# kserve/kserve

Measured on AMD Instinct MI355X. Metric: output tok/s, llama-3-8b /v1/completions decode, higher is better.
Workload: dtype bfloat16; 1 GPU; model=llama-3-8b, global_batch=1536, seq_len=512, parallelism=dp1, kv_block_size=16, hipgraph=True, kv_cache_dtype=auto

## Files before the change

### build_hip.py

```python
#!/usr/bin/env python3

import os
import subprocess
import sys

REPO = os.path.dirname(os.path.abspath(__file__))
CSRC = os.path.join(REPO, "kserve_amd", "ops", "csrc")
BUILD = os.path.join(REPO, "build", "hip")
OUT_SO = os.path.join(REPO, "kserve_amd_C.so")

HIPCC = os.environ.get("HIPCC", "/opt/rocm/bin/hipcc")
ARCH = os.environ.get("PYTORCH_ROCM_ARCH", "gfx950")

KERNEL_SOURCES = [
    "rmsnorm.hip",
    "layernorm.hip",
    "activation.hip",
    "rope.hip",
    "kv_cache.hip",
    "attention_decode.hip",
    "attention_prefill.hip",
    "sampling.hip",
    "skinny_gemm.hip",
    "w8_gemm.hip",
    "gemm8.hip",
    "mfma_probe.hip",
]


def run(cmd):
    print("+", " ".join(cmd), flush=True)
    subprocess.check_call(cmd)


def newer(src, dst):
    return not os.path.exists(dst) or os.path.getmtime(src) > os.path.getmtime(dst)


def build(force: bool = False) -> str:
    import torch
    import sysconfig

    os.makedirs(BUILD, exist_ok=True)
    torch_dir = os.path.dirname(torch.__file__)
    torch_inc = [
        os.path.join(torch_dir, "include"),
        os.path.join(torch_dir, "include", "torch", "csrc", "api", "include"),
    ]
    py_inc = sysconfig.get_paths()["include"]

    common_h = os.path.join(CSRC, "common.h")
    layouts_h = os.path.join(CSRC, "mfma_layouts.h")
    objs = []
    for src in KERNEL_SOURCES:
        src_path = os.path.join(CSRC, src)
        obj = os.path.join(BUILD, src.replace(".hip", ".o"))
        objs.append(obj)
        if force or newer(src_path, obj) or newer(common_h, obj) or newer(layouts_h, obj):
            run([
                HIPCC, "-c", src_path, "-o", obj,
                f"--offload-arch={ARCH}", "-O3", "-std=c++17", "-fPIC",
                "-ffast-math",
            ])

    bind_src = os.path.join(CSRC, "bindings.cpp")
    bind_obj = os.path.join(BUILD, "bindings.o")
    if force or newer(bind_src, bind_obj):
        cmd = [
            HIPCC, "-c", bind_src, "-o", bind_obj,
            "-O2", "-std=c++17", "-fPIC",
            "-D_GLIBCXX_USE_CXX11_ABI=1",
            "-DTORCH_EXTENSION_NAME=kserve_amd_C",
            "-DUSE_ROCM", "-D__HIP_PLATFORM_AMD__",
            "-DTORCH_API_INCLUDE_EXTENSION_H",
            f"-I{py_inc}",
        ]
        cmd += [f"-I{d}" for d in torch_inc]
        run(cmd)
    objs.append(bind_obj)

    if force or any(newer(o, OUT_SO) for o in objs):
        run([
            HIPCC, "-shared", "-o", OUT_SO, *objs,
            f"-L{os.path.join(torch_dir, 'lib')}",
            "-ltorch", "-ltorch_cpu", "-ltorch_python", "-lc10",
            "-ltorch_hip", "-lc10_hip", "-lamdhip64",
            f"-Wl,-rpath,{os.path.join(torch_dir, 'lib')}",
        ])
    print(f"built {OUT_SO}")
    return OUT_SO


if __name__ == "__main__":
    build(force="--force" in sys.argv)
```

### kserve_amd/ops/__init__.py

```python

from __future__ import annotations

from typing import Optional, Tuple

import torch

from kserve_amd.errors import NoNativeExtension
from kserve_amd.ops import torch_ref

_C = None
_IMPORT_ERROR: Optional[str] = None
try:
    import kserve_amd_C as _C
except ImportError as e:
    _IMPORT_ERROR = str(e)


def has_native() -> bool:
    return _C is not None


def _native(op: str):
    if _C is None:
        raise NoNativeExtension(op, f"(import error: {_IMPORT_ERROR})")
    return _C


def rms_norm(x: torch.Tensor, weight: torch.Tensor, eps: float) -> torch.Tensor:
    if x.is_cuda:
        out = torch.empty_like(x)
        _native("rms_norm").rms_norm(out, x, weight, eps)
        return out
    return torch_ref.rms_norm(x, weight, eps)


def fused_add_rms_norm(
    x: torch.Tensor, residual: torch.Tensor, weight: torch.Tensor, eps: float
) -> Tuple[torch.Tensor, torch.Tensor]:
    if x.is_cuda:
        _native("fused_add_rms_norm").fused_add_rms_norm(x, residual, weight, eps)
        return x, residual
    return torch_ref.fused_add_rms_norm(x, residual, weight, eps)


def silu_and_mul(x: torch.Tensor) -> torch.Tensor:
    if x.is_cuda:
        d = x.shape[-1] // 2
        out = torch.empty(
            (*x.shape[:-1], d), dtype=x.dtype, device=x.device
        )
        _native("silu_and_mul").silu_and_mul(out, x)
        return out
    return torch_ref.silu_and_mul(x)


def rotary_embedding(
    positions: torch.Tensor,
    q: torch.Tensor,
    k: torch.Tensor,
    cos_sin_cache: torch.Tensor,
) -> Tuple[torch.Tensor, torch.Tensor]:
    if q.is_cuda:
        _native("rotary_embedding").rotary_embedding(positions, q, k, cos_sin_cache)
        return q, k
    return torch_ref.rotary_embedding(positions, q, k, cos_sin_cache)


def reshape_and_cache(
    k: torch.Tensor,
    v: torch.Tensor,
    k_cache: torch.Tensor,
    v_cache: torch.Tensor,
    slot_mapping: torch.Tensor,
) -> None:
    if k.is_cuda:
        _native("reshape_and_cache").reshape_and_cache(
            k, v, k_cache, v_cache, slot_mapping
        )
        return
    torch_ref.reshape_and_cache(k, v, k_cache, v_cache, slot_mapping)


def paged_attention_decode(
    q: torch.Tensor,
    k_cache: torch.Tensor,
    v_cache: torch.Tensor,
    block_tables: torch.Tensor,
    context_lens: torch.Tensor,
    scale: float,
    out: Optional[torch.Tensor] = None,
    window: int = 0,
) -> torch.Tensor:
    if q.is_cuda:
        if out is None:
            out = torch.empty_like(q)
        _native("paged_attention_decode").paged_attention_decode(
            out, q, k_cache, v_cache, block_tables, context_lens, scale,
            window,
        )
        return out
    return torch_ref.paged_attention_decode(
        q, k_cache, v_cache, block_tables, context_lens, scale,
        window=window,
    )


def flash_prefill_varlen(
    q: torch.Tensor,
    k: torch.Tensor,
    v: torch.Tensor,
    cu_seqlens: torch.Tensor,
    max_seqlen: int,
    scale: float,
    window: int = 0,
) -> torch.Tensor:
    if q.is_cuda:
        out = torch.empty_like(q)
        _native("flash_prefill").flash_prefill_varlen(
            out, q, k, v, cu_seqlens, int(max_seqlen), scale,
            causal=True, window=window,
        )
        return out
    return torch_ref.flash_prefill_varlen(
        q, k, v, cu_seqlens, scale, causal=True, window=window
    )


def context_attention_varlen(
    q: torch.Tensor,
    k_cache: torch.Tensor,
    v_cache: torch.Tensor,
    block_tables: torch.Tensor,
    cu_seqlens_q: torch.Tensor,
    context_lens: torch.Tensor,
    max_q_len: int,
    scale: float,
    window: int = 0,
) -> torch.Tensor:
    if q.is_cuda:
        out = torch.empty_like(q)
        _native("context_prefill").context_prefill_varlen(
            out, q, k_cache, v_cache, block_tables, context_lens,
            cu_seqlens_q, int(max_q_len), scale, window
        )
        return out
    return torch_ref.context_attention_varlen(
        q, k_cache, v_cache, block_tables, cu_seqlens_q, context_lens, scale,
        window=window,
    )


def greedy_sample(logits: torch.Tensor) -> torch.Tensor:
    if logits.is_cuda:
        out = torch.empty(
            logits.shape[0], dtype=torch.int64, device=logits.device
        )
        _native("greedy_sample").greedy_sample(out, logits)
        return out
    return torch_ref.greedy_sample(logits)


def random_sample(
    logits: torch.Tensor,
    temperatures: torch.Tensor,
    top_p: torch.Tensor,
    top_k: torch.Tensor,
    seeds: Optional[torch.Tensor] = None,
    generator: Optional[torch.Generator] = None,
    min_p: Optional[torch.Tensor] = None,
) -> torch.Tensor:
    has_min_p = min_p is not None and bool((min_p > 0).any())
    if logits.is_cuda and seeds is not None and not has_min_p:
        out = torch.empty(
            logits.shape[0], dtype=torch.int64, device=logits.device
        )
        needs_trunc = bool((top_p < 1.0).any()) or bool((top_k > 0).any())
        if needs_trunc:
            _native("random_sample").topk_topp_sample(
                out, logits, temperatures, top_p, top_k.to(torch.int32), seeds
            )
        else:
            _native("random_sample").gumbel_sample(
                out, logits, temperatures, top_k.to(torch.int32), seeds
            )
        return out
    return torch_ref.random_sample(
        logits, temperatures, top_p, top_k, generator=generator, min_p=min_p
    )


def linear(x: torch.Tensor, weight: torch.Tensor, bias: Optional[torch.Tensor] = None) -> torch.Tensor:
    import torch.nn.functional as F

    if (
        _C is not None
        and x.is_cuda
        and bias is None
        and x.dim() == 2
        and 0 < x.shape[0] <= 64
        and weight.shape[0] % 64 == 0
        and weight.shape[0] <= 8192
        and weight.shape[1] % 64 == 0
        and weight.shape[1] <= 8192
        and x.stride(1) == 1
    ):
        out = torch.empty(
            (x.shape[0], weight.shape[0]), dtype=x.dtype, device=x.device
        )
        _C.skinny_gemm(out, x, weight)
        return out
    return F.linear(x, weight, bias)


W8_MAX_TOKENS = 128

_W8_SCRATCH: dict = {}


def w8_scratch_numel(out_features: int, in_features: int) -> int:
    return -(-out_features // 2) * in_features


def reserve_w8_scratch(device, out_features: int, in_features: int) -> None:
    device = torch.device(device)
    if device.type != "cuda":
        return
    if device.index is None:
        device = torch.device("cuda", torch.cuda.current_device())
    numel = w8_scratch_numel(out_features, in_features)
    buf = _W8_SCRATCH.get(device)
    if buf is None or buf.numel() < numel:
        _W8_SCRATCH[device] = None
        _W8_SCRATCH[device] = torch.empty(
            numel, dtype=torch.bfloat16, device=device
        )


def _w8_scratch(device, out_features: int, in_features: int) -> torch.Tensor:
    buf = _W8_SCRATCH.get(device)
    if buf is None or buf.numel() < w8_scratch_numel(out_features, in_features):
        if torch.cuda.is_current_stream_capturing():
            raise RuntimeError(
                "fp8 dequant scratch too small during graph capture; "
                "call ops.reserve_w8_scratch when the weight is quantized"
            )
        reserve_w8_scratch(device, out_features, in_features)
        buf = _W8_SCRATCH[device]
    return buf


def linear_w8(
    x: torch.Tensor,
    qweight: torch.Tensor,
    scale: torch.Tensor,
    bias: Optional[torch.Tensor] = None,
) -> torch.Tensor:
    if not x.is_cuda:
# ... 86 lines not shown
```

### kserve_amd/ops/csrc/attention_decode.hip

```cpp
#include "common.h"
#include "mfma_layouts.h"

#define NEG_INF (-1e30f)

namespace {

constexpr int PAGE = 16;
constexpr int NWAVES = 4;

typedef __bf16 bf16x2v_t __attribute__((ext_vector_type(2)));

template <int D, int HPW, int OCC = 1, bool PB = false, bool D2 = false,
          bool V4 = false, bool MQ = false>
__global__ __launch_bounds__(256, OCC) void paged_attention_kernel(
    short* __restrict__ out,
    const short* __restrict__ q,
    const short* __restrict__ k_cache,
    const short* __restrict__ v_cache,
    const int* __restrict__ block_tables,
    const int* __restrict__ context_lens,
    const float scale,
    const int num_kv_heads,
    const int group,
    const int max_blocks,
// ... 798 lines not shown
        }
      }
    }
  }

#pragma unroll
  for (int g = 0; g < GROUP; ++g) {
    if (lane == 0) {
      lds_ml[wave][g][0] = m[g];
      lds_ml[wave][g][1] = l[g];
    }
#pragma unroll
    for (int a = 0; a < ACC; ++a)
      lds_acc[wave][g][lane * ACC + a] = acc[g][a];
  }
  __syncthreads();
  for (int g = wave; g < GROUP; g += NWAVES) {
    float m_all = NEG_INF;
#pragma unroll
    for (int w = 0; w < NWAVES; ++w) m_all = fmaxf(m_all, lds_ml[w][g][0]);
    float l_all = 0.f;
    float a_all[ACC];
#pragma unroll
    for (int a = 0; a < ACC; ++a) a_all[a] = 0.f;
#pragma unroll
    for (int w = 0; w < NWAVES; ++w) {
      const float wgt = __expf(lds_ml[w][g][0] - m_all);
      l_all += wgt * lds_ml[w][g][1];
#pragma unroll
      for (int a = 0; a < ACC; ++a)
        a_all[a] += wgt * lds_acc[w][g][lane * ACC + a];
    }
    const int head = kv_head * GROUP + g;
    if (n_splits == 1) {
      const float inv_l = (l_all > 0.f) ? 1.f / l_all : 0.f;
      short* op = out + ((long)seq * num_heads + head) * D + lane * ACC;
#pragma unroll
      for (int a = 0; a < ACC; ++a)
        op[a] = float_to_bf16_bits(a_all[a] * inv_l);
    } else {
      float* po = part_out +
                  (((long)seq * num_heads + head) * n_splits + split) * D +
                  lane * ACC;
#pragma unroll
      for (int a = 0; a < ACC; ++a) po[a] = a_all[a];
      if (lane == 0) {
        float* ml =
            part_ml + (((long)seq * num_heads + head) * n_splits + split) * 2;
        ml[0] = m_all;
        ml[1] = l_all;
      }
    }
  }
}

template <int D>
__global__ void paged_attention_reduce_kernel(
    short* __restrict__ out,
    const float* __restrict__ part_out,
    const float* __restrict__ part_ml,
    const long total_sh, const int n_splits) {
  constexpr int ACC = D / 64;
  const long sh = blockIdx.x * (long)(blockDim.x >> 6) + (threadIdx.x >> 6);
  const int lane = threadIdx.x & 63;
  if (sh >= total_sh) return;
  const float* ml_base = part_ml + sh * n_splits * 2;
  float m = NEG_INF;
  for (int sp = 0; sp < n_splits; ++sp) m = fmaxf(m, ml_base[sp * 2]);
  float l = 0.f;
  float acc[ACC];
#pragma unroll
  for (int a = 0; a < ACC; ++a) acc[a] = 0.f;
  for (int sp = 0; sp < n_splits; ++sp) {
    const float ms = ml_base[sp * 2];
    const float ls = ml_base[sp * 2 + 1];
    if (ls <= 0.f || ms <= NEG_INF) continue;
    const float w = __expf(ms - m);
    l += ls * w;
    const float* po = part_out + (sh * n_splits + sp) * D + lane * ACC;
#pragma unroll
    for (int a = 0; a < ACC; ++a) acc[a] += w * po[a];
  }
  const float inv_l = (l > 0.f) ? 1.f / l : 0.f;
  short* op = out + sh * D + lane * ACC;
#pragma unroll
  for (int a = 0; a < ACC; ++a) op[a] = float_to_bf16_bits(acc[a] * inv_l);
}

}


namespace {
inline hipError_t launch_split_reduce(void* out, void* part_out,
                                      void* part_ml, int num_seqs,
                                      int num_heads, int head_dim,
                                      int n_splits, hipStream_t stream) {
  if (n_splits <= 1) return hipSuccess;
  const long sh = (long)num_seqs * num_heads;
  const int wpb = 4;
  dim3 rgrid((unsigned)((sh + wpb - 1) / wpb));
  if (head_dim == 128) {
    hipLaunchKernelGGL((paged_attention_reduce_kernel<128>), rgrid,
                       dim3(wpb * 64), 0, stream, (short*)out,
                       (const float*)part_out, (const float*)part_ml, sh,
                       n_splits);
  } else {
    hipLaunchKernelGGL((paged_attention_reduce_kernel<64>), rgrid,
                       dim3(wpb * 64), 0, stream, (short*)out,
                       (const float*)part_out, (const float*)part_ml, sh,
                       n_splits);
  }
  HIP_CHECK_KERNEL();
  return hipSuccess;
}
}

extern "C" hipError_t ks_paged_attention_decode_fp8(
    void* out, const void* q, const void* k_cache, const void* v_cache,
    const void* block_tables, const void* context_lens, float scale,
    int num_seqs, int num_heads, int num_kv_heads, int head_dim,
    int max_blocks, int block_size, long q_row_stride, int n_splits,
    void* part_out, void* part_ml, int window, hipStream_t stream) {
  if (block_size != PAGE || head_dim != 128) return hipErrorInvalidValue;
  const int group = num_heads / num_kv_heads;
  if (group > NWAVES) return hipErrorInvalidValue;
  if (n_splits < 1) n_splits = 1;
  dim3 grid(num_kv_heads, num_seqs, n_splits);
  static const bool cvtb = [] {
    const char* e = getenv("KS_FP8_CVTB");
    return e == nullptr || e[0] != '0';
  }();
  if (cvtb) {
    hipLaunchKernelGGL((paged_attention_fp8_kernel<128, true>), grid,
                       dim3(256), 0, stream, (short*)out, (const short*)q,
                       (const unsigned char*)k_cache,
                       (const unsigned char*)v_cache,
                       (const int*)block_tables, (const int*)context_lens,
                       scale, num_kv_heads, group, max_blocks, q_row_stride,
                       n_splits, (float*)part_out, (float*)part_ml, window);
  } else {
    hipLaunchKernelGGL((paged_attention_fp8_kernel<128, false>), grid,
                       dim3(256), 0, stream, (short*)out, (const short*)q,
                       (const unsigned char*)k_cache,
                       (const unsigned char*)v_cache,
                       (const int*)block_tables, (const int*)context_lens,
                       scale, num_kv_heads, group, max_blocks, q_row_stride,
                       n_splits, (float*)part_out, (float*)part_ml, window);
  }
  HIP_CHECK_KERNEL();
  return launch_split_reduce(out, part_out, part_ml, num_seqs, num_heads,
                             head_dim, n_splits, stream);
}

extern "C" hipError_t ks_paged_attention_decode(
    void* out, const void* q, const void* k_cache, const void* v_cache,
    const void* block_tables, const void* context_lens, float scale,
    int num_seqs, int num_heads, int num_kv_heads, int head_dim,
    int max_blocks, int block_size, long q_row_stride, int n_splits,
    void* part_out, void* part_ml, int window, hipStream_t stream) {
  if (block_size != PAGE) return hipErrorInvalidValue;
  const int group = num_heads / num_kv_heads;
  const int hpw = (group + NWAVES - 1) / NWAVES;
  if (hpw > 2) return hipErrorInvalidValue;
  if (n_splits < 1) n_splits = 1;
  dim3 grid(num_kv_heads, num_seqs, n_splits);
  dim3 block(256);

  static const bool use_ws = [] {
    const char* e = getenv("KS_ATTN_WS");
    return e != nullptr && e[0] == '1';
  }();
  const bool pow2_group =
      group == 1 || group == 2 || group == 4 || group == 8;
  if (use_ws && pow2_group && head_dim == 128) {
#define LAUNCH_WS(GG)                                                       \
  hipLaunchKernelGGL((paged_attention_ws_kernel<128, GG>), grid, block, 0,  \
                     stream, (short*)out, (const short*)q,                  \
                     (const short*)k_cache, (const short*)v_cache,          \
                     (const int*)block_tables, (const int*)context_lens,    \
                     scale, num_kv_heads, max_blocks, q_row_stride,         \
                     n_splits, (float*)part_out, (float*)part_ml, window)
    if (group == 1) LAUNCH_WS(1);
    else if (group == 2) LAUNCH_WS(2);
    else if (group == 4) LAUNCH_WS(4);
    else LAUNCH_WS(8);
#undef LAUNCH_WS
    HIP_CHECK_KERNEL();
    return launch_split_reduce(out, part_out, part_ml, num_seqs, num_heads,
                               head_dim, n_splits, stream);
  }

  static const bool use_h2 = [] {
    const char* e = getenv("KS_ATTN_H2");
    return e != nullptr && e[0] == '1';
  }();
  if (use_h2 && group == 4 && head_dim == 128) {
    hipLaunchKernelGGL((paged_attention_kernel<128, 2>), grid, dim3(128), 0,
                       stream, (short*)out, (const short*)q,
                       (const short*)k_cache, (const short*)v_cache,
                       (const int*)block_tables, (const int*)context_lens,
                       scale, num_kv_heads, group, max_blocks, q_row_stride,
                       n_splits, (float*)part_out, (float*)part_ml, window);
    HIP_CHECK_KERNEL();
    return launch_split_reduce(out, part_out, part_ml, num_seqs, num_heads,
                               head_dim, n_splits, stream);
  }

  static const bool use_mq = [] {
    const char* e = getenv("KS_ATTN_MQ");
    return e != nullptr && e[0] == '1';
  }();
  if (use_mq && hpw == 1 && head_dim == 128) {
    hipLaunchKernelGGL(
        (paged_attention_kernel<128, 1, 1, true, false, true, true>), grid,
        block, 0, stream, (short*)out, (const short*)q,
        (const short*)k_cache, (const short*)v_cache,
        (const int*)block_tables, (const int*)context_lens, scale,
        num_kv_heads, group, max_blocks, q_row_stride, n_splits,
        (float*)part_out, (float*)part_ml, window);
    HIP_CHECK_KERNEL();
    return launch_split_reduce(out, part_out, part_ml, num_seqs, num_heads,
                               head_dim, n_splits, stream);
  }

  static const bool use_u2 = [] {
    const char* e = getenv("KS_ATTN_U2");
    return e != nullptr && e[0] == '1';
  }();
  if (use_u2 && hpw == 1 && head_dim == 128) {
    hipLaunchKernelGGL((paged_attention_u2_kernel<128>), grid, block, 0,
                       stream, (short*)out, (const short*)q,
                       (const short*)k_cache, (const short*)v_cache,
                       (const int*)block_tables, (const int*)context_lens,
                       scale, num_kv_heads, group, max_blocks, q_row_stride,
                       n_splits, (float*)part_out, (float*)part_ml, window);
    HIP_CHECK_KERNEL();
    return launch_split_reduce(out, part_out, part_ml, num_seqs, num_heads,
                               head_dim, n_splits, stream);
  }
  static const int occ = [] {
    const char* e = getenv("KS_ATTN_OCC");
    return e ? atoi(e) : 0;
  }();
  static const bool use_pb = [] {
    const char* e = getenv("KS_ATTN_PB");
    return e == nullptr || e[0] != '0';
  }();
  static const int v4_mode = [] {
    const char* e = getenv("KS_ATTN_V4");
    return e ? (e[0] == '1' ? 1 : 0) : -1;
  }();
  const bool use_v4 =
      v4_mode == 1 || (v4_mode == -1 && num_seqs > 128);
  static const bool v4_d2 = [] {
    const char* e = getenv("KS_ATTN_V4D2");
    return e != nullptr && e[0] == '1';
  }();
  if (use_v4 && hpw == 1 && head_dim == 128) {
    if (v4_d2) {
      hipLaunchKernelGGL(
          (paged_attention_kernel<128, 1, 1, true, true, true>), grid, block,
          0, stream, (short*)out, (const short*)q, (const short*)k_cache,
          (const short*)v_cache, (const int*)block_tables,
          (const int*)context_lens, scale, num_kv_heads, group, max_blocks,
          q_row_stride, n_splits, (float*)part_out, (float*)part_ml, window);
    } else {
      hipLaunchKernelGGL(
          (paged_attention_kernel<128, 1, 1, true, false, true>), grid,
          block, 0, stream, (short*)out, (const short*)q,
          (const short*)k_cache, (const short*)v_cache,
          (const int*)block_tables, (const int*)context_lens, scale,
          num_kv_heads, group, max_blocks, q_row_stride, n_splits,
          (float*)part_out, (float*)part_ml, window);
    }
    HIP_CHECK_KERNEL();
    return launch_split_reduce(out, part_out, part_ml, num_seqs, num_heads,
                               head_dim, n_splits, stream);
  }
  static const int d2_mode = [] {
    const char* e = getenv("KS_ATTN_D2");
    return e ? (e[0] == '1' ? 1 : 0) : -1;
  }();
  const bool use_d2 =
      d2_mode == 1 || (d2_mode == -1 && num_seqs <= 128);
  if (use_d2 && hpw == 1 && head_dim == 128) {
    hipLaunchKernelGGL((paged_attention_kernel<128, 1, 1, true, true>), grid,
                       block, 0, stream, (short*)out, (const short*)q,
                       (const short*)k_cache, (const short*)v_cache,
                       (const int*)block_tables, (const int*)context_lens,
                       scale, num_kv_heads, group, max_blocks, q_row_stride,
                       n_splits, (float*)part_out, (float*)part_ml, window);
    HIP_CHECK_KERNEL();
    return launch_split_reduce(out, part_out, part_ml, num_seqs, num_heads,
                               head_dim, n_splits, stream);
  }
  if (use_pb && hpw == 1 && head_dim == 128) {
    hipLaunchKernelGGL((paged_attention_kernel<128, 1, 1, true>), grid, block,
                       0, stream, (short*)out, (const short*)q,
                       (const short*)k_cache, (const short*)v_cache,
                       (const int*)block_tables, (const int*)context_lens,
                       scale, num_kv_heads, group, max_blocks, q_row_stride,
                       n_splits, (float*)part_out, (float*)part_ml, window);
    HIP_CHECK_KERNEL();
    return launch_split_reduce(out, part_out, part_ml, num_seqs, num_heads,
                               head_dim, n_splits, stream);
  }
  if (occ >= 5 && hpw == 1 && head_dim == 128) {
    if (occ >= 6) {
      hipLaunchKernelGGL((paged_attention_kernel<128, 1, 6>), grid, block, 0,
                         stream, (short*)out, (const short*)q,
                         (const short*)k_cache, (const short*)v_cache,
                         (const int*)block_tables, (const int*)context_lens,
                         scale, num_kv_heads, group, max_blocks, q_row_stride,
                         n_splits, (float*)part_out, (float*)part_ml, window);
    } else {
      hipLaunchKernelGGL((paged_attention_kernel<128, 1, 5>), grid, block, 0,
                         stream, (short*)out, (const short*)q,
                         (const short*)k_cache, (const short*)v_cache,
                         (const int*)block_tables, (const int*)context_lens,
// ... 29 lines not shown
```

### kserve_amd/ops/csrc/bindings.cpp

```cpp
#include <torch/extension.h>

#include <c10/hip/HIPStream.h>

#include <hip/hip_runtime.h>

extern "C" {
hipError_t ks_rms_norm(void*, const void*, const void*, float, int, int,
                       hipStream_t);
hipError_t ks_fused_add_rms_norm(void*, void*, const void*, float, int, int,
                                 hipStream_t);
hipError_t ks_silu_and_mul(void*, const void*, int, int, hipStream_t);
hipError_t ks_rotary_embedding(void*, void*, const void*, const void*, int,
                               int, int, int, long, long, hipStream_t);
hipError_t ks_reshape_and_cache(const void*, const void*, void*, void*,
                                const void*, int, int, int, int, long, long,
                                hipStream_t);
hipError_t ks_paged_attention_decode(void*, const void*, const void*,
                                     const void*, const void*, const void*,
                                     float, int, int, int, int, int, int,
                                     long, int, void*, void*, int,
                                     hipStream_t);
hipError_t ks_flash_prefill_varlen(void*, const void*, const void*,
                                   const void*, const void*, int, int, int,
                                   int, int, float, long, long, long, int,
                                   int, hipStream_t);
hipError_t ks_context_prefill_varlen(void*, const void*, const void*,
                                     const void*, const void*, const void*,
                                     const void*, int, int, int, int, int,
                                     int, float, long, int, int,
                                     hipStream_t);
hipError_t ks_paged_attention_decode_fp8(void*, const void*, const void*,
                                         const void*, const void*,
                                         const void*, float, int, int, int,
                                         int, int, int, long, int, void*,
                                         void*, int, hipStream_t);
hipError_t ks_reshape_and_cache_fp8(const void*, const void*, void*, void*,
                                    const void*, int, int, int, int, long,
                                    long, hipStream_t);
hipError_t ks_layer_norm(void*, const void*, const void*, const void*, float,
                         int, int, hipStream_t);
hipError_t ks_fused_add_layer_norm(void*, const void*, const void*,
                                   const void*, const void*, float, int, int,
                                   hipStream_t);
hipError_t ks_gelu(void*, const void*, long, hipStream_t);
hipError_t ks_greedy_sample(void*, const void*, int, int, hipStream_t);
hipError_t ks_gumbel_sample(void*, const void*, const void*, const void*,
                            const void*, int, int, hipStream_t);
hipError_t ks_topk_topp_sample(void*, const void*, const void*, const void*,
                               const void*, const void*, int, int,
                               hipStream_t);
hipError_t ks_mfma_probe(void*, const void*, const void*, hipStream_t);
hipError_t ks_skinny_gemm(void*, void*, const void*, const void*, int, int,
                          int, long, hipStream_t);
hipError_t ks_gemm8(void*, const void*, const void*, int, int, int, int,
                    hipStream_t);
int ks_skinny_gemm_w8_nsplit(int, int);
hipError_t ks_skinny_gemm_w8(void*, void*, const void*, const void*,
                             const void*, int, int, int, long, hipStream_t);
hipError_t ks_dequant_fp8_rows(void*, const void*, const void*, long, int,
                               hipStream_t);
}

namespace {

hipStream_t current_stream() {
  return c10::hip::getCurrentHIPStream().stream();
}

void check_hip(hipError_t err, const char* op) {
  TORCH_CHECK(err == hipSuccess, op, " failed: ", hipGetErrorString(err));
}

#define CHECK_BF16_CONTIG(t)                                       \
  TORCH_CHECK((t).scalar_type() == at::kBFloat16, #t " must be bf16"); \
  TORCH_CHECK((t).is_contiguous(), #t " must be contiguous");      \
  TORCH_CHECK((t).is_cuda(), #t " must be on GPU")

#define CHECK_KV_CACHE(t)                                               \
  TORCH_CHECK((t).scalar_type() == at::kBFloat16 ||                       \
                  (t).scalar_type() == at::kFloat8_e4m3fn,                \
              #t " must be bf16 or fp8_e4m3");                            \
  TORCH_CHECK((t).is_contiguous(), #t " must be contiguous");             \
  TORCH_CHECK((t).is_cuda(), #t " must be on GPU")

#define CHECK_BF16_ROWS(t)                                              \
  TORCH_CHECK((t).scalar_type() == at::kBFloat16, #t " must be bf16");  \
  TORCH_CHECK((t).is_cuda(), #t " must be on GPU");                     \
  TORCH_CHECK((t).dim() == 3 && (t).stride(2) == 1 &&                   \
                  (t).stride(1) == (t).size(2),                         \
              #t " inner dims must be dense")

void rms_norm(at::Tensor& out, at::Tensor& input, at::Tensor& weight,
              double eps) {
  CHECK_BF16_CONTIG(out);
  CHECK_BF16_CONTIG(input);
  CHECK_BF16_CONTIG(weight);
  int hidden = input.size(-1);
  int rows = input.numel() / hidden;
  check_hip(ks_rms_norm(out.data_ptr(), input.data_ptr(), weight.data_ptr(),
                        (float)eps, rows, hidden, current_stream()),
            "rms_norm");
}

void fused_add_rms_norm(at::Tensor& x, at::Tensor& residual, at::Tensor& weight,
                        double eps) {
  CHECK_BF16_CONTIG(x);
  CHECK_BF16_CONTIG(residual);
  int hidden = x.size(-1);
  int rows = x.numel() / hidden;
  check_hip(
      ks_fused_add_rms_norm(x.data_ptr(), residual.data_ptr(),
                            weight.data_ptr(), (float)eps, rows, hidden,
                            current_stream()),
      "fused_add_rms_norm");
}

void silu_and_mul(at::Tensor& out, at::Tensor& input) {
  CHECK_BF16_CONTIG(out);
  CHECK_BF16_CONTIG(input);
  int d = out.size(-1);
  TORCH_CHECK(input.size(-1) == 2 * d, "input last dim must be 2*out");
  int rows = out.numel() / d;
  check_hip(ks_silu_and_mul(out.data_ptr(), input.data_ptr(), rows, d,
                            current_stream()),
            "silu_and_mul");
}

void rotary_embedding(at::Tensor& positions, at::Tensor& q, at::Tensor& k,
                      at::Tensor& cos_sin_cache) {
  CHECK_BF16_ROWS(q);
  CHECK_BF16_ROWS(k);
  TORCH_CHECK(positions.scalar_type() == at::kLong, "positions must be int64");
  TORCH_CHECK(cos_sin_cache.scalar_type() == at::kFloat,
              "cos_sin_cache must be fp32");
  int T = q.size(0);
  int Hq = q.size(1);
  int Hk = k.size(1);
  int D = q.size(2);
  check_hip(ks_rotary_embedding(q.data_ptr(), k.data_ptr(),
                                positions.data_ptr(), cos_sin_cache.data_ptr(),
                                T, Hq, Hk, D, (long)q.stride(0),
                                (long)k.stride(0), current_stream()),
            "rotary_embedding");
}

void reshape_and_cache(at::Tensor& k, at::Tensor& v, at::Tensor& k_cache,
                       at::Tensor& v_cache, at::Tensor& slot_mapping) {
  CHECK_BF16_ROWS(k);
  CHECK_BF16_ROWS(v);
  CHECK_KV_CACHE(k_cache);
  CHECK_KV_CACHE(v_cache);
  TORCH_CHECK(slot_mapping.scalar_type() == at::kInt, "slot_mapping int32");
  int T = k.size(0);
  int Hkv = k.size(1);
  int D = k.size(2);
  int block_size = k_cache.size(2);
  if (k_cache.scalar_type() == at::kFloat8_e4m3fn) {
    check_hip(ks_reshape_and_cache_fp8(k.data_ptr(), v.data_ptr(),
                                       k_cache.data_ptr(), v_cache.data_ptr(),
                                       slot_mapping.data_ptr(), T, Hkv, D,
                                       block_size, (long)k.stride(0),
                                       (long)v.stride(0), current_stream()),
              "reshape_and_cache_fp8");
    return;
  }
  check_hip(ks_reshape_and_cache(k.data_ptr(), v.data_ptr(),
                                 k_cache.data_ptr(), v_cache.data_ptr(),
                                 slot_mapping.data_ptr(), T, Hkv, D,
                                 block_size, (long)k.stride(0),
                                 (long)v.stride(0), current_stream()),
            "reshape_and_cache");
}

void paged_attention_decode(at::Tensor& out, at::Tensor& q,
                            at::Tensor& k_cache, at::Tensor& v_cache,
                            at::Tensor& block_tables, at::Tensor& context_lens,
                            double scale, int64_t window) {
  CHECK_BF16_CONTIG(out);
  CHECK_BF16_ROWS(q);
  CHECK_KV_CACHE(k_cache);
  CHECK_KV_CACHE(v_cache);
  TORCH_CHECK(block_tables.scalar_type() == at::kInt, "block_tables int32");
  TORCH_CHECK(context_lens.scalar_type() == at::kInt, "context_lens int32");
  const bool fp8 = k_cache.scalar_type() == at::kFloat8_e4m3fn;
  int S = q.size(0);
  int H = q.size(1);
  int D = q.size(2);
  int Hkv = k_cache.size(1);
  int block_size = k_cache.size(2);
  int max_blocks = block_tables.size(1);
  int n_splits = 1;
  long base_wgs = (long)S * Hkv;
  const int grp = H / Hkv;
  static const int split_override = [] {
    const char* e = getenv("KS_ATTN_SPLIT");
    return e ? atoi(e) : 0;
  }();
  if (split_override > 0) {
    n_splits = split_override;
  } else if (grp <= 4 && base_wgs <= 512) {
    n_splits = (int)(2048 / base_wgs);
    if (n_splits < 2) n_splits = 2;
    if (n_splits > 8) n_splits = 8;
  } else if (base_wgs < 512) {
    n_splits = (int)((512 + base_wgs - 1) / base_wgs);
    if (n_splits > 16) n_splits = 16;
  }
  if (n_splits > 1) {
    int max_split_blocks = (max_blocks + n_splits - 1) / n_splits;
    if (max_split_blocks < 1) n_splits = 1;
  }
  at::Tensor part_out, part_ml;
  void *po = nullptr, *pml = nullptr;
  if (n_splits > 1) {
    auto opts = at::TensorOptions().dtype(at::kFloat).device(q.device());
    part_out = at::empty({S, H, n_splits, D}, opts);
    part_ml = at::empty({S, H, n_splits, 2}, opts);
    po = part_out.data_ptr();
    pml = part_ml.data_ptr();
  }
  if (fp8) {
    TORCH_CHECK(H / Hkv <= 4 && D == 128,
                "fp8 KV decode supports D=128 and GQA group <= 4");
    check_hip(ks_paged_attention_decode_fp8(
                  out.data_ptr(), q.data_ptr(), k_cache.data_ptr(),
                  v_cache.data_ptr(), block_tables.data_ptr(),
                  context_lens.data_ptr(), (float)scale, S, H, Hkv, D,
                  max_blocks, block_size, (long)q.stride(0), n_splits, po,
                  pml, (int)window, current_stream()),
              "paged_attention_decode_fp8");
    return;
  }
  check_hip(ks_paged_attention_decode(
                out.data_ptr(), q.data_ptr(), k_cache.data_ptr(),
                v_cache.data_ptr(), block_tables.data_ptr(),
                context_lens.data_ptr(), (float)scale, S, H, Hkv, D,
                max_blocks, block_size, (long)q.stride(0), n_splits, po, pml,
                (int)window, current_stream()),
            "paged_attention_decode");
}

void flash_prefill_varlen(at::Tensor& out, at::Tensor& q, at::Tensor& k,
                          at::Tensor& v, at::Tensor& cu_seqlens,
                          int64_t max_seqlen, double scale,
                          bool causal = true, int64_t window = 0) {
  CHECK_BF16_CONTIG(out);
  CHECK_BF16_ROWS(q);
  CHECK_BF16_ROWS(k);
  CHECK_BF16_ROWS(v);
  TORCH_CHECK(cu_seqlens.scalar_type() == at::kInt, "cu_seqlens int32");
  int num_seqs = cu_seqlens.size(0) - 1;
  int Hq = q.size(1);
  int Hkv = k.size(1);
  int D = q.size(2);
  check_hip(ks_flash_prefill_varlen(out.data_ptr(), q.data_ptr(), k.data_ptr(),
                                    v.data_ptr(), cu_seqlens.data_ptr(),
                                    num_seqs, (int)max_seqlen, Hq, Hkv, D,
                                    (float)scale, (long)q.stride(0),
                                    (long)k.stride(0), (long)v.stride(0),
                                    causal ? 1 : 0, (int)window,
                                    current_stream()),
            "flash_prefill_varlen");
}

void context_prefill_varlen(at::Tensor& out, at::Tensor& q,
                            at::Tensor& k_cache, at::Tensor& v_cache,
                            at::Tensor& block_tables, at::Tensor& ctx_lens,
                            at::Tensor& cu_seqlens_q, int64_t max_q_len,
                            double scale, int64_t window) {
  CHECK_BF16_CONTIG(out);
  CHECK_BF16_ROWS(q);
  CHECK_KV_CACHE(k_cache);
  CHECK_KV_CACHE(v_cache);
  TORCH_CHECK(block_tables.scalar_type() == at::kInt, "block_tables int32");
  TORCH_CHECK(block_tables.is_contiguous(), "block_tables contiguous");
  TORCH_CHECK(ctx_lens.scalar_type() == at::kInt, "ctx_lens int32");
  TORCH_CHECK(cu_seqlens_q.scalar_type() == at::kInt, "cu_seqlens_q int32");
  TORCH_CHECK(k_cache.size(2) == 16, "block_size must be 16");
  int num_seqs = cu_seqlens_q.size(0) - 1;
  int Hq = q.size(1);
  int Hkv = k_cache.size(1);
  int D = q.size(2);
  int fp8 = k_cache.scalar_type() == at::kFloat8_e4m3fn ? 1 : 0;
  check_hip(ks_context_prefill_varlen(
                out.data_ptr(), q.data_ptr(), k_cache.data_ptr(),
                v_cache.data_ptr(), block_tables.data_ptr(),
                ctx_lens.data_ptr(), cu_seqlens_q.data_ptr(), num_seqs,
                (int)max_q_len, Hq, Hkv, D, (int)block_tables.size(1),
                (float)scale, (long)q.stride(0), fp8, (int)window,
                current_stream()),
            "context_prefill_varlen");
}

void layer_norm(at::Tensor& out, at::Tensor& input, at::Tensor& weight,
                at::Tensor& bias, double eps) {
  CHECK_BF16_CONTIG(out);
  CHECK_BF16_CONTIG(input);
  int hidden = input.size(-1);
  int rows = input.numel() / hidden;
  check_hip(ks_layer_norm(out.data_ptr(), input.data_ptr(), weight.data_ptr(),
                          bias.data_ptr(), (float)eps, rows, hidden,
                          current_stream()),
            "layer_norm");
}

void fused_add_layer_norm(at::Tensor& out, at::Tensor& input,
                          at::Tensor& residual, at::Tensor& weight,
                          at::Tensor& bias, double eps) {
  CHECK_BF16_CONTIG(out);
  CHECK_BF16_CONTIG(input);
  CHECK_BF16_CONTIG(residual);
  int hidden = input.size(-1);
  int rows = input.numel() / hidden;
  check_hip(ks_fused_add_layer_norm(out.data_ptr(), input.data_ptr(),
                                    residual.data_ptr(), weight.data_ptr(),
                                    bias.data_ptr(), (float)eps, rows, hidden,
                                    current_stream()),
            "fused_add_layer_norm");
}

void gelu(at::Tensor& out, at::Tensor& input) {
  CHECK_BF16_CONTIG(out);
  CHECK_BF16_CONTIG(input);
  check_hip(ks_gelu(out.data_ptr(), input.data_ptr(), input.numel(),
                    current_stream()),
            "gelu");
}

void greedy_sample(at::Tensor& out, at::Tensor& logits) {
  CHECK_BF16_CONTIG(logits);
  TORCH_CHECK(out.scalar_type() == at::kLong, "out int64");
  check_hip(ks_greedy_sample(out.data_ptr(), logits.data_ptr(),
                             logits.size(0), logits.size(1),
                             current_stream()),
            "greedy_sample");
}

void gumbel_sample(at::Tensor& out, at::Tensor& logits,
                   at::Tensor& temperatures, at::Tensor& top_k,
                   at::Tensor& seeds) {
  CHECK_BF16_CONTIG(logits);
  TORCH_CHECK(out.scalar_type() == at::kLong, "out int64");
  TORCH_CHECK(temperatures.scalar_type() == at::kFloat, "temps fp32");
  TORCH_CHECK(seeds.scalar_type() == at::kLong, "seeds int64");
  check_hip(ks_gumbel_sample(out.data_ptr(), logits.data_ptr(),
                             temperatures.data_ptr(), top_k.data_ptr(),
                             seeds.data_ptr(), logits.size(0), logits.size(1),
                             current_stream()),
            "gumbel_sample");
}

void topk_topp_sample(at::Tensor& out, at::Tensor& logits,
                      at::Tensor& temperatures, at::Tensor& top_p,
                      at::Tensor& top_k, at::Tensor& seeds) {
  CHECK_BF16_CONTIG(logits);
  TORCH_CHECK(out.scalar_type() == at::kLong, "out int64");
  TORCH_CHECK(temperatures.scalar_type() == at::kFloat, "temps fp32");
  TORCH_CHECK(top_p.scalar_type() == at::kFloat, "top_p fp32");
  TORCH_CHECK(top_k.scalar_type() == at::kInt, "top_k int32");
  TORCH_CHECK(seeds.scalar_type() == at::kLong, "seeds int64");
  check_hip(ks_topk_topp_sample(out.data_ptr(), logits.data_ptr(),
                                temperatures.data_ptr(), top_p.data_ptr(),
                                top_k.data_ptr(), seeds.data_ptr(),
                                logits.size(0), logits.size(1),
                                current_stream()),
            "topk_topp_sample");
}

void skinny_gemm(at::Tensor& out, at::Tensor& x, at::Tensor& w) {
  CHECK_BF16_CONTIG(out);
  CHECK_BF16_CONTIG(w);
  TORCH_CHECK(x.scalar_type() == at::kBFloat16 && x.is_cuda() &&
                  x.stride(1) == 1,
              "x must be bf16 row-dense");
  int N = x.size(0);
  int K = x.size(1);
  int M = w.size(0);
  TORCH_CHECK(w.size(1) == K, "shape mismatch");
  at::Tensor ws;
  void* wsp = nullptr;
  int nsplit = 1;
  int feat_wgs = M / 64;
  while (feat_wgs * nsplit < 768 && nsplit < 8 && (K / (nsplit * 2)) >= 64)
    nsplit *= 2;
  if (nsplit > 1) {
    ws = at::empty({(long)nsplit * N * M},
                   at::TensorOptions().dtype(at::kBFloat16).device(x.device()));
    wsp = ws.data_ptr();
  }
  check_hip(ks_skinny_gemm(out.data_ptr(), wsp, x.data_ptr(), w.data_ptr(),
                           M, K, N, (long)x.stride(0), current_stream()),
            "skinny_gemm");
}

#define CHECK_FP8_WEIGHT(q, scale)                                        \
  TORCH_CHECK((q).scalar_type() == at::kFloat8_e4m3fn && (q).is_cuda() && \
                  (q).dim() == 2 && (q).is_contiguous(),                  \
              #q " must be a contiguous 2-D fp8_e4m3fn GPU tensor");      \
  TORCH_CHECK((scale).scalar_type() == at::kFloat && (scale).is_cuda() && \
                  (scale).is_contiguous() &&                              \
                  (scale).numel() == (q).size(0),                         \
              #scale " must be f32 [out_features] on GPU")

void skinny_gemm_w8(at::Tensor& out, at::Tensor& x, at::Tensor& qweight,
                    at::Tensor& scale) {
  CHECK_BF16_CONTIG(out);
  CHECK_FP8_WEIGHT(qweight, scale);
  TORCH_CHECK(x.scalar_type() == at::kBFloat16 && x.is_cuda() &&
                  x.dim() == 2 && x.stride(1) == 1,
              "x must be bf16 row-dense");
  int N = x.size(0);
  int K = x.size(1);
  int M = qweight.size(0);
  TORCH_CHECK(qweight.size(1) == K && out.dim() == 2 && out.size(0) == N &&
                  out.size(1) == M,
              "shape mismatch");
  TORCH_CHECK(N >= 1 && N <= 256 && M % 64 == 0 && K % 64 == 0,
              "skinny_gemm_w8 needs 1 <= N <= 256, M % 64 == 0, K % 64 == 0");
  at::Tensor ws;
  void* wsp = nullptr;
  const int nsplit = ks_skinny_gemm_w8_nsplit(M, K);
  if (nsplit > 1) {
    ws = at::empty({(long)nsplit * N * M},
                   at::TensorOptions().dtype(at::kBFloat16).device(x.device()));
    wsp = ws.data_ptr();
  }
  check_hip(ks_skinny_gemm_w8(out.data_ptr(), wsp, x.data_ptr(),
                              qweight.data_ptr(), scale.data_ptr(), M, K, N,
                              (long)x.stride(0), current_stream()),
            "skinny_gemm_w8");
}

void dequant_fp8_rows(at::Tensor& out, at::Tensor& qweight,
                      at::Tensor& scale) {
  CHECK_BF16_CONTIG(out);
  CHECK_FP8_WEIGHT(qweight, scale);
  TORCH_CHECK(out.numel() == qweight.numel(), "shape mismatch");
  check_hip(ks_dequant_fp8_rows(out.data_ptr(), qweight.data_ptr(),
                                scale.data_ptr(), (long)qweight.size(0),
                                (int)qweight.size(1), current_stream()),
            "dequant_fp8_rows");
}

void gemm8(at::Tensor& d, at::Tensor& a, at::Tensor& w, int64_t swizzle) {
  CHECK_BF16_CONTIG(d);
  CHECK_BF16_CONTIG(a);
  CHECK_BF16_CONTIG(w);
  int M = a.size(0), K = a.size(1), N = w.size(0);
  TORCH_CHECK(w.size(1) == K && d.size(0) == M && d.size(1) == N,
              "shape mismatch");
  check_hip(ks_gemm8(d.data_ptr(), a.data_ptr(), w.data_ptr(), M, N, K,
                     (int)swizzle, current_stream()),
            "gemm8");
}

void mfma_probe(at::Tensor& c, at::Tensor& a, at::Tensor& b) {
  check_hip(ks_mfma_probe(c.data_ptr(), a.data_ptr(), b.data_ptr(),
                          current_stream()),
            "mfma_probe");
}

}

PYBIND11_MODULE(TORCH_EXTENSION_NAME, m) {
  m.def("rms_norm", &rms_norm, "RMSNorm (bf16, CDNA4)");
  m.def("fused_add_rms_norm", &fused_add_rms_norm,
        "fused residual-add + RMSNorm, in-place");
  m.def("silu_and_mul", &silu_and_mul, "SwiGLU activation");
  m.def("rotary_embedding", &rotary_embedding, "neox RoPE in-place");
  m.def("reshape_and_cache", &reshape_and_cache, "KV page scatter");
  m.def("paged_attention_decode", &paged_attention_decode,
        "paged decode attention (GQA, split-context)");
  m.def("flash_prefill_varlen", &flash_prefill_varlen,
        "MFMA flash attention (varlen GQA, causal or bidirectional)",
        pybind11::arg("out"), pybind11::arg("q"), pybind11::arg("k"),
        pybind11::arg("v"), pybind11::arg("cu_seqlens"),
        pybind11::arg("max_seqlen"), pybind11::arg("scale"),
        pybind11::arg("causal") = true, pybind11::arg("window") = 0);
  m.def("context_prefill_varlen", &context_prefill_varlen,
        "MFMA prefill attention against the paged KV cache (chunked prefill)");
  m.def("layer_norm", &layer_norm, "LayerNorm (bf16)");
  m.def("fused_add_layer_norm", &fused_add_layer_norm,
        "residual-add + LayerNorm");
  m.def("gelu", &gelu, "erf GELU");
  m.def("greedy_sample", &greedy_sample, "argmax sampling");
  m.def("gumbel_sample", &gumbel_sample, "Gumbel-max temperature sampling");
  m.def("topk_topp_sample", &topk_topp_sample,
        "fused top-k/top-p + Gumbel-max sampler (radix-histogram select)");
  m.def("skinny_gemm", &skinny_gemm, "decode GEMM (N<=256, MFMA streaming)");
  m.def("skinny_gemm_w8", &skinny_gemm_w8,
        "decode GEMM, fp8 e4m3 weights x bf16 activations (N<=256)");
  m.def("dequant_fp8_rows", &dequant_fp8_rows,
        "fp8 e4m3 rows * per-row scale -> bf16");
  m.def("gemm8", &gemm8,
        "EXPERIMENTAL 8-phase 256x256 MFMA GEMM (round-2 candidate)");
  m.def("mfma_probe", &mfma_probe, "MFMA layout probe (tests)");
}
```

Measured before the change: 30130 tok/s.

## Add GQA-packed MFMA paged decode attention kernel and auto-route group-8 batches

Measured after the change: 30020 tok/s (median of 3 runs). No clear change (-0.3%).

```diff
diff --git a/build_hip.py b/build_hip.py
--- a/build_hip.py
+++ b/build_hip.py
@@ -19,6 +19,7 @@
     "rope.hip",
     "kv_cache.hip",
     "attention_decode.hip",
+    "attention_decode_gq.hip",
     "attention_prefill.hip",
     "sampling.hip",
     "skinny_gemm.hip",
diff --git a/kserve_amd/ops/__init__.py b/kserve_amd/ops/__init__.py
--- a/kserve_amd/ops/__init__.py
+++ b/kserve_amd/ops/__init__.py
@@ -103,6 +103,25 @@
         q, k_cache, v_cache, block_tables, context_lens, scale,
         window=window,
     )
+
+
+def paged_attention_decode_gq(
+    q: torch.Tensor,
+    k_cache: torch.Tensor,
+    v_cache: torch.Tensor,
+    block_tables: torch.Tensor,
+    context_lens: torch.Tensor,
+    scale: float,
+    out: Optional[torch.Tensor] = None,
+) -> torch.Tensor:
+    if not q.is_cuda:
+        raise ValueError("paged_attention_decode_gq is a GPU kernel")
+    if out is None:
+        out = torch.empty(q.shape, dtype=q.dtype, device=q.device)
+    _native("paged_attention_decode_gq").paged_attention_decode_gq(
+        out, q, k_cache, v_cache, block_tables, context_lens, scale
+    )
+    return out
 
 
 def flash_prefill_varlen(
diff --git a/kserve_amd/ops/csrc/attention_decode.hip b/kserve_amd/ops/csrc/attention_decode.hip
--- a/kserve_amd/ops/csrc/attention_decode.hip
+++ b/kserve_amd/ops/csrc/attention_decode.hip
@@ -974,6 +974,18 @@
                              head_dim, n_splits, stream);
 }
 
+extern "C" hipError_t ks_paged_attention_decode_gq(
+    void* out, const void* q, const void* k_cache, const void* v_cache,
+    const void* block_tables, const void* context_lens, float scale,
+    int num_seqs, int num_heads, int num_kv_heads, int head_dim,
+    int max_blocks, int block_size, long q_row_stride, hipStream_t stream);
+
+namespace {
+inline bool gq_auto(int num_seqs, int group) {
+  return group == 8 && num_seqs >= 64;
+}
+}
+
 extern "C" hipError_t ks_paged_attention_decode(
     void* out, const void* q, const void* k_cache, const void* v_cache,
     const void* block_tables, const void* context_lens, float scale,
@@ -983,10 +995,25 @@
   if (block_size != PAGE) return hipErrorInvalidValue;
   const int group = num_heads / num_kv_heads;
   const int hpw = (group + NWAVES - 1) / NWAVES;
-  if (hpw > 2) return hipErrorInvalidValue;
   if (n_splits < 1) n_splits = 1;
   dim3 grid(num_kv_heads, num_seqs, n_splits);
   dim3 block(256);
+
+  static const int gq_mode = [] {
+    const char* e = getenv("KS_ATTN_GQ");
+    return e ? (e[0] == '1' ? 1 : 0) : -1;
+  }();
+  if (gq_mode != 0 && window == 0 && n_splits == 1 && head_dim == 128 &&
+      group >= 1 && group <= 16 && num_heads == group * num_kv_heads &&
+      q_row_stride % 8 == 0 &&
+      (((uintptr_t)q | (uintptr_t)k_cache | (uintptr_t)v_cache) & 15) == 0 &&
+      (gq_mode == 1 || gq_auto(num_seqs, group))) {
+    return ks_paged_attention_decode_gq(
+        out, q, k_cache, v_cache, block_tables, context_lens, scale, num_seqs,
+        num_heads, num_kv_heads, head_dim, max_blocks, block_size,
+        q_row_stride, stream);
+  }
+  if (hpw > 2) return hipErrorInvalidValue;
 
   static const bool use_ws = [] {
     const char* e = getenv("KS_ATTN_WS");
diff --git a/kserve_amd/ops/csrc/attention_decode_gq.hip b/kserve_amd/ops/csrc/attention_decode_gq.hip
--- /dev/null
+++ b/kserve_amd/ops/csrc/attention_decode_gq.hip
@@ -0,0 +1,245 @@
+#include "common.h"
+#include "mfma_layouts.h"
+
+#define NEG_INF (-1e30f)
+
+namespace {
+
+constexpr int PAGE = 16;
+constexpr int HD = 128;
+constexpr int NWAVES = 4;
+constexpr int GQ_MAX_GROUP = 16;
+constexpr int PAGE_BYTES = PAGE * HD * 2;
+constexpr int WAVE_LDS = 2 * PAGE_BYTES;
+constexpr int ML_BYTES = NWAVES * GQ_MAX_GROUP * 2 * 4;
+
+typedef short short4v_t __attribute__((ext_vector_type(4)));
+typedef __attribute__((address_space(3))) short4v_t lds_short4v_t;
+
+__device__ __forceinline__ float gq_mul_f32_unpacked(float a, float b) {
+  float r;
+  asm("v_mul_f32 %0, %1, %2" : "=v"(r) : "v"(a), "v"(b));
+  return r;
+}
+
+__device__ __forceinline__ bf16x8_t as_bf16x8(short8_t v) {
+  return __builtin_bit_cast(bf16x8_t, v);
+}
+
+__device__ __forceinline__ short4v_t lds_read_tr(const char* p) {
+  return __builtin_amdgcn_ds_read_tr16_b64_v4i16((lds_short4v_t*)p);
+}
+
+__global__ __launch_bounds__(256, 4) void paged_attention_gq_kernel(
+    short* __restrict__ out,
+    const short* __restrict__ q,
+    const short* __restrict__ k_cache,
+    const short* __restrict__ v_cache,
+    const int* __restrict__ block_tables,
+    const int* __restrict__ context_lens,
+    const float scale_log2e,
+    const int num_kv_heads,
+    const int group,
+    const int max_blocks,
+    const long q_row_stride
+) {
+  __shared__ __attribute__((aligned(16))) char smem[NWAVES * WAVE_LDS + ML_BYTES];
+
+  const int kv_head = blockIdx.x;
+  const int seq = blockIdx.y;
+  const int ctx = context_lens[seq];
+  if (ctx <= 0) return;
+  const int lane = threadIdx.x & 63;
+  const int wave = __builtin_amdgcn_readfirstlane(threadIdx.x >> 6);
+  const int r = lane & 15;
+  const int g = lane >> 4;
+  const int num_heads = num_kv_heads * group;
+  const int nblocks = (ctx + PAGE - 1) / PAGE;
+  const int npairs = (nblocks + 1) >> 1;
+
+  bf16x8_t bq[4];
+  {
+    const int hr = min(r, group - 1);
+    const short* qp = q + (long)seq * q_row_stride +
+                      (long)(kv_head * group + hr) * HD + 32 * g;
+#pragma unroll
+    for (int ki = 0; ki < 4; ++ki) {
+      short8_t t = *reinterpret_cast<const short8_t*>(qp + 8 * ki);
+      if (r >= group) t = short8_t{0, 0, 0, 0, 0, 0, 0, 0};
+      bq[ki] = as_bf16x8(t);
+    }
+  }
+
+  float m = NEG_INF, l = 0.f;
+  f32x4_t o[8];
+#pragma unroll
+  for (int mb = 0; mb < 8; ++mb) o[mb] = f32x4_t{0.f, 0.f, 0.f, 0.f};
+
+  char* vimg = smem + wave * WAVE_LDS;
+  const char* tr_base = vimg + (4 * g + (r >> 2)) * (HD * 2) + (r & 3) * 8;
+  const int* bt = block_tables + (long)seq * max_blocks;
+  const int k_lane_off = r * HD + 32 * g;
+  const int v_lane_off = lane * 8;
+
+  for (int pi = wave; pi < npairs; pi += NWAVES) {
+    const int i0 = 2 * pi;
+    const int i1 = min(i0 + 1, nblocks - 1);
+    const long base0 = ((long)bt[i0] * num_kv_heads + kv_head) * (PAGE * HD);
+    const long base1 = ((long)bt[i1] * num_kv_heads + kv_head) * (PAGE * HD);
+
+    short8_t ka[2][4];
+    short8_t vr[2][4];
+#pragma unroll
+    for (int ki = 0; ki < 4; ++ki) {
+      ka[0][ki] = *reinterpret_cast<const short8_t*>(
+          k_cache + base0 + k_lane_off + 8 * ki);
+      ka[1][ki] = *reinterpret_cast<const short8_t*>(
+          k_cache + base1 + k_lane_off + 8 * ki);
+    }
+#pragma unroll
+    for (int i = 0; i < 4; ++i) {
+      vr[0][i] = *reinterpret_cast<const short8_t*>(
+          v_cache + base0 + v_lane_off + 512 * i);
+      vr[1][i] = *reinterpret_cast<const short8_t*>(
+          v_cache + base1 + v_lane_off + 512 * i);
+    }
+
+    f32x4_t c0 = f32x4_t{0.f, 0.f, 0.f, 0.f};
+    f32x4_t c1 = f32x4_t{0.f, 0.f, 0.f, 0.f};
+#pragma unroll
+    for (int ki = 0; ki < 4; ++ki) {
+      c0 = mfma16x16x32(as_bf16x8(ka[0][ki]), bq[ki], c0);
+      c1 = mfma16x16x32(as_bf16x8(ka[1][ki]), bq[ki], c1);
+    }
+
+#pragma unroll
+    for (int i = 0; i < 4; ++i) {
+      *reinterpret_cast<short8_t*>(vimg + lane * 16 + 1024 * i) = vr[0][i];
+      *reinterpret_cast<short8_t*>(vimg + PAGE_BYTES + lane * 16 + 1024 * i) =
+          vr[1][i];
+    }
+
+    const int tok0 = i0 * PAGE + 4 * g;
+    float s0[4], s1[4];
+    float mx = NEG_INF;
+#pragma unroll
+    for (int j = 0; j < 4; ++j) {
+      s0[j] = (tok0 + j < ctx) ? c0[j] * scale_log2e : NEG_INF;
+      s1[j] = (tok0 + PAGE + j < ctx) ? c1[j] * scale_log2e : NEG_INF;
+      mx = fmaxf(mx, fmaxf(s0[j], s1[j]));
+    }
+    mx = fmaxf(mx, __shfl_xor(mx, 16, 64));
+    mx = fmaxf(mx, __shfl_xor(mx, 32, 64));
+    const float m_new = fmaxf(m, mx);
+    const float rescale = __builtin_amdgcn_exp2f(m - m_new);
+    float psum = 0.f;
+#pragma unroll
+    for (int j = 0; j < 4; ++j) {
+      s0[j] = (s0[j] > NEG_INF) ? __builtin_amdgcn_exp2f(s0[j] - m_new) : 0.f;
+      s1[j] = (s1[j] > NEG_INF) ? __builtin_amdgcn_exp2f(s1[j] - m_new) : 0.f;
+      psum += s0[j] + s1[j];
+    }
+    psum += __shfl_xor(psum, 16, 64);
+    psum += __shfl_xor(psum, 32, 64);
+    l = l * rescale + psum;
+    m = m_new;
+
+    bf16x8_t bp, bp_lo;
+#pragma unroll
+    for (int j = 0; j < 4; ++j) {
+      bp[j] = (__bf16)s0[j];
+      bp[4 + j] = (__bf16)s1[j];
+      bp_lo[j] = (__bf16)(s0[j] - (float)bp[j]);
+      bp_lo[4 + j] = (__bf16)(s1[j] - (float)bp[4 + j]);
+    }
+
+    float rescale_v;
+    asm("s_nop 1\n\tv_mov_b32 %0, %1" : "=v"(rescale_v) : "v"(rescale));
+#pragma unroll
+    for (int mb = 0; mb < 8; ++mb) {
+#pragma unroll
+      for (int reg = 0; reg < 4; ++reg)
+        o[mb][reg] = gq_mul_f32_unpacked(o[mb][reg], rescale_v);
+    }
+
+#pragma unroll
+    for (int mb = 0; mb < 8; ++mb) {
+      const short4v_t a0 = lds_read_tr(tr_base + 32 * mb);
+      const short4v_t a1 = lds_read_tr(tr_base + PAGE_BYTES + 32 * mb);
+      const short8_t av =
+          __builtin_shufflevector(a0, a1, 0, 1, 2, 3, 4, 5, 6, 7);
+      o[mb] = mfma16x16x32(as_bf16x8(av), bp, o[mb]);
+      o[mb] = mfma16x16x32(as_bf16x8(av), bp_lo, o[mb]);
+    }
+  }
+
+  float* obuf = reinterpret_cast<float*>(vimg);
+#pragma unroll
+  for (int mb = 0; mb < 8; ++mb) {
+    const int ch = (4 * mb + g) ^ r;
+    *reinterpret_cast<f32x4_t*>(obuf + r * HD + ch * 4) = o[mb];
+  }
+  float* ml = reinterpret_cast<float*>(smem + NWAVES * WAVE_LDS);
+  if (g == 0) {
+    ml[(wave * GQ_MAX_GROUP + r) * 2] = m;
+    ml[(wave * GQ_MAX_GROUP + r) * 2 + 1] = l;
+  }
+  __syncthreads();
+
+  for (int idx = threadIdx.x; idx < group * (HD / 2); idx += 256) {
+    const int h = idx >> 6;
+    const int dp = idx & 63;
+    float mw[NWAVES];
+    float m_all = NEG_INF;
+#pragma unroll
+    for (int w = 0; w < NWAVES; ++w) {
+      mw[w] = ml[(w * GQ_MAX_GROUP + h) * 2];
+      m_all = fmaxf(m_all, mw[w]);
+    }
+    float l_all = 0.f, a0 = 0.f, a1 = 0.f;
+    const int off = h * HD + (((dp >> 1) ^ h) << 2) + ((dp & 1) << 1);
+#pragma unroll
+    for (int w = 0; w < NWAVES; ++w) {
+      const float wgt = __builtin_amdgcn_exp2f(mw[w] - m_all);
+      l_all += wgt * ml[(w * GQ_MAX_GROUP + h) * 2 + 1];
+      const float2_t v = *reinterpret_cast<const float2_t*>(
+          reinterpret_cast<const float*>(smem + w * WAVE_LDS) + off);
+      a0 += wgt * v[0];
+      a1 += wgt * v[1];
+    }
+    const float inv_l = (l_all > 0.f) ? 1.f / l_all : 0.f;
+    const unsigned int lo = (unsigned short)float_to_bf16_bits(a0 * inv_l);
+    const unsigned int hi = (unsigned short)float_to_bf16_bits(a1 * inv_l);
+    unsigned int* op = reinterpret_cast<unsigned int*>(
+        out + ((long)seq * num_heads + kv_head * group + h) * HD + 2 * dp);
+    *op = lo | (hi << 16);
+  }
+}
+
+}
+
+extern "C" hipError_t ks_paged_attention_decode_gq(
+    void* out, const void* q, const void* k_cache, const void* v_cache,
+    const void* block_tables, const void* context_lens, float scale,
+    int num_seqs, int num_heads, int num_kv_heads, int head_dim,
+    int max_blocks, int block_size, long q_row_stride, hipStream_t stream) {
+  if (block_size != PAGE || head_dim != HD) return hipErrorInvalidValue;
+  if (num_kv_heads < 1 || num_heads % num_kv_heads != 0)
+    return hipErrorInvalidValue;
+  const int group = num_heads / num_kv_heads;
+  if (group < 1 || group > GQ_MAX_GROUP) return hipErrorInvalidValue;
+  if (num_seqs < 1 || num_seqs > 65535 || max_blocks < 1)
+    return hipErrorInvalidValue;
+  if (q_row_stride % 8 != 0 || ((uintptr_t)q & 15) != 0 ||
+      ((uintptr_t)k_cache & 15) != 0 || ((uintptr_t)v_cache & 15) != 0 ||
+      ((uintptr_t)out & 3) != 0)
+    return hipErrorInvalidValue;
+  dim3 grid(num_kv_heads, num_seqs);
+  hipLaunchKernelGGL(paged_attention_gq_kernel, grid, dim3(256), 0, stream,
+                     (short*)out, (const short*)q, (const short*)k_cache,
+                     (const short*)v_cache, (const int*)block_tables,
+                     (const int*)context_lens, scale * 1.4426950408889634f,
+                     num_kv_heads, group, max_blocks, q_row_stride);
+  HIP_CHECK_KERNEL();
+  return hipSuccess;
+}
diff --git a/kserve_amd/ops/csrc/bindings.cpp b/kserve_amd/ops/csrc/bindings.cpp
--- a/kserve_amd/ops/csrc/bindings.cpp
+++ b/kserve_amd/ops/csrc/bindings.cpp
@@ -20,6 +20,10 @@
                                      float, int, int, int, int, int, int,
                                      long, int, void*, void*, int,
                                      hipStream_t);
+hipError_t ks_paged_attention_decode_gq(void*, const void*, const void*,
+                                        const void*, const void*, const void*,
+                                        float, int, int, int, int, int, int,
+                                        long, hipStream_t);
 hipError_t ks_flash_prefill_varlen(void*, const void*, const void*,
                                    const void*, const void*, int, int, int,
                                    int, int, float, long, long, long, int,
@@ -240,6 +244,45 @@
             "paged_attention_decode");
 }
 
+void paged_attention_decode_gq(at::Tensor& out, at::Tensor& q,
+                               at::Tensor& k_cache, at::Tensor& v_cache,
+                               at::Tensor& block_tables,
+                               at::Tensor& context_lens, double scale) {
+  CHECK_BF16_CONTIG(out);
+  CHECK_BF16_ROWS(q);
+  CHECK_BF16_CONTIG(k_cache);
+  CHECK_BF16_CONTIG(v_cache);
+  TORCH_CHECK(block_tables.scalar_type() == at::kInt && block_tables.is_cuda() &&
+                  block_tables.dim() == 2 && block_tables.is_contiguous(),
+              "block_tables must be contiguous int32 [S, max_blocks] on GPU");
+  TORCH_CHECK(context_lens.scalar_type() == at::kInt && context_lens.is_cuda() &&
+                  context_lens.is_contiguous(),
+              "context_lens must be contiguous int32 on GPU");
+  TORCH_CHECK(k_cache.dim() == 4 && v_cache.sizes() == k_cache.sizes(),
+              "k_cache/v_cache must be [blocks, Hkv, page, D]");
+  int S = q.size(0);
+  int H = q.size(1);
+  int D = q.size(2);
+  int Hkv = k_cache.size(1);
+  int block_size = k_cache.size(2);
+  TORCH_CHECK(out.dim() == 3 && out.size(0) == S && out.size(1) == H &&
+                  out.size(2) == D,
+              "out must be [S, H, D]");
+  TORCH_CHECK(block_tables.size(0) == S && context_lens.numel() == S,
+              "block_tables/context_lens must have one row per sequence");
+  TORCH_CHECK(D == 128 && k_cache.size(3) == 128 && block_size == 16,
+              "GQ decode needs head_dim 128 and page size 16");
+  TORCH_CHECK(Hkv >= 1 && H % Hkv == 0 && H / Hkv >= 1 && H / Hkv <= 16,
+              "GQ decode needs 1 <= GQA group <= 16");
+  check_hip(ks_paged_attention_decode_gq(
+                out.data_ptr(), q.data_ptr(), k_cache.data_ptr(),
+                v_cache.data_ptr(), block_tables.data_ptr(),
+                context_lens.data_ptr(), (float)scale, S, H, Hkv, D,
+                (int)block_tables.size(1), block_size, (long)q.stride(0),
+                current_stream()),
+            "paged_attention_decode_gq");
+}
+
 void flash_prefill_varlen(at::Tensor& out, at::Tensor& q, at::Tensor& k,
                           at::Tensor& v, at::Tensor& cu_seqlens,
                           int64_t max_seqlen, double scale,
@@ -471,6 +514,8 @@
   m.def("reshape_and_cache", &reshape_and_cache, "KV page scatter");
   m.def("paged_attention_decode", &paged_attention_decode,
         "paged decode attention (GQA, split-context)");
+  m.def("paged_attention_decode_gq", &paged_attention_decode_gq,
+        "paged decode attention, one wave per KV page pair, GQA heads on MFMA");
   m.def("flash_prefill_varlen", &flash_prefill_varlen,
         "MFMA flash attention (varlen GQA, causal or bidirectional)",
         pybind11::arg("out"), pybind11::arg("q"), pybind11::arg("k"),
```
